# Vicky0522/TokensGen

Measured on AMD Instinct MI355X. Metric: DiT denoising steps/sec, CogVideoX-5B To2V 720x480 (CFG-batched 13-frame FIFO window: DiT fwd + CFG + 13 DPM updates), higher is better.
Workload: dtype bf16; 1 GPU; To2V FIFO window step, CogVideoX-5B 42 layers D=3072, 226 text + 17550 video + 480 vip tokens, CFG batch 2, DPM-solver++; layers=42, exchange=none

## Files before the change

include/tokensgen_hip.h:

```cpp
#ifndef TOKENSGEN_HIP_H
#define TOKENSGEN_HIP_H

#include <stdint.h>

#ifdef __cplusplus
extern "C" {
#endif
#if defined(__GNUC__)
#pragma GCC visibility push(default)
#endif

typedef struct ihipStream_t* hipStream_t;

#define TG_MAX_GROUPS 16

typedef struct tg_group_table {
    const void*    mod;
    long           mod_ld;
    long           mod_batch_stride;
    const uint8_t* tok_group;
    int32_t        row[TG_MAX_GROUPS];
    int32_t        shift_col[TG_MAX_GROUPS];
    int32_t        scale_col[TG_MAX_GROUPS];
    int32_t        gate_col[TG_MAX_GROUPS];
// ... 21 lines not shown

int tg_gemm_bf16_qkv(const void* A1, long strideA1, const void* W1, const void* bias1, void* C1, long strideC1, int M1, void* Vt1, long vt_ld1,
                     const void* A2, long strideA2, const void* W2, const void* bias2, void* C2, long strideC2, int M2, void* Vt2, long vt_ld2,
                     long lda, long ldw, long ldc, int N, int K, int batch, int v_col0, hipStream_t stream);

int tg_gemm_bf16_lora(const void* A, long lda, long strideA, const void* W, long ldw, const void* bias,
                      const void* T, long ldt, long strideT, const void* B, long ldb, float scale,
                      void* C, long ldc, long strideC, int M, int N, int K, int R, int batch, hipStream_t stream);

long tg_gemm_kernel(int M, int N, int K, long lda, long ldw);

int tg_adaln_modulate(const void* x, long ldx, long strideX, void* y, long ldy, long strideY,
                      const void* ln_weight, const void* ln_bias, float eps, int tokens, int dim, int batch,
                      int modulate, const tg_group_table* g, hipStream_t stream);

int tg_qk_layernorm_rope(void* x, long ld, long strideB, int tokens, int heads, int batch,
                         const void* ln_weight, const void* ln_bias, float eps,
                         int start0, int len0, const float* cos0, const float* sin0,
                         int start1, int len1, const float* cos1, const float* sin1, float out_scale, hipStream_t stream);

int tg_qk_layernorm_rope_pair(void* xq, void* xk, long ld, long strideB, int tokens, int heads, int batch,
                              const void* q_weight, const void* q_bias, const void* k_weight, const void* k_bias, float eps,
                              int start0, int len0, const float* cos0, const float* sin0,
                              int start1, int len1, const float* cos1, const float* sin1, float q_scale, float k_scale,
                              hipStream_t stream);

long tg_qk_kmax_ws_floats(int tokens, int heads, int batch);
int tg_qk_layernorm_rope_pair_kmax(void* xq, void* xk, long ld, long strideB, int tokens, int heads, int batch,
                                   const void* q_weight, const void* q_bias, const void* k_weight, const void* k_bias, float eps,
                                   int start0, int len0, const float* cos0, const float* sin0,
                                   int start1, int len1, const float* cos1, const float* sin1, float q_scale, float k_scale,
                                   float* k_norm2_max, float* ws, hipStream_t stream);

int tg_qk_layernorm_rope_pair_out(const void* xq, const void* xk, long ld, long strideB, void* yq, void* yk, long y_ld, long y_strideB, int tokens, int heads,
                                  int batch, const void* q_weight, const void* q_bias, const void* k_weight, const void* k_bias, float eps,
                                  int start0, int len0, const float* cos0, const float* sin0, int start1, int len1, const float* cos1, const float* sin1,
                                  float q_scale, float k_scale, float* k_norm2_max, float* ws, hipStream_t stream);

int tg_transpose_v(const void* v, long ld, long strideB, int key_start, int n_keys, int heads, int batch,
                   void* vt, long ldvt, hipStream_t stream);

int tg_attention_fwd(const void* q1, long q1_ld, long q1_strideB,
                     const void* k1, long k1_ld, long k1_strideB, const void* vt1, long vt1_ld, int nk1,
                     const void* q2, long q2_ld, long q2_strideB,
                     const void* k2, long k2_ld, long k2_strideB, const void* vt2, long vt2_ld, int nk2,
                     float seg2_scale, void* out, long out_ld, long out_strideB,
                     int nq, int heads, int batch, float scale, int k_prescaled, hipStream_t stream);

typedef struct tg_attn_segment {
    const void* q; long q_ld, q_strideB;
    const void* k; long k_ld, k_strideB;
    const void* vt; long vt_ld;
// ... 248 lines not shown
```

tokensgen_amd/csrc/norm.hip:

```cpp
#include "common.h"
#include "tokensgen_hip.h"

namespace {

template <int CHUNKS>
__global__ __launch_bounds__(256) void adaln_kernel(const bf16_t* __restrict__ x, long ldx, long sxb,
                                                    bf16_t* __restrict__ y, long ldy, long syb,
                                                    const bf16_t* __restrict__ w, const bf16_t* __restrict__ bvec,
                                                    float eps, int tokens, int dim, int batch, int modulate,
                                                    tg_group_table g) {
    const int lane = threadIdx.x & 63;
    const long row = (long)blockIdx.x * 4 + (threadIdx.x >> 6);
    if (row >= (long)tokens * batch) return;
    const int b = (int)(row / tokens), t = (int)(row % tokens);
    const bf16_t* xr = x + (long)b * sxb + (long)t * ldx;
    bf16_t* yr = y + (long)b * syb + (long)t * ldy;
    const int nvec = dim >> 3;

    uint4 raw[CHUNKS];
    float s = 0.f;
#pragma unroll
    for (int c = 0; c < CHUNKS; ++c) {
        const int v = c * 64 + lane;
        raw[c] = (v < nvec) ? *(const uint4*)(xr + v * 8) : uint4{0, 0, 0, 0};
// ... 39 lines not shown
            su[0] = sv.x; su[1] = sv.y; su[2] = sv.z; su[3] = sv.w;
            hu[0] = hv.x; hu[1] = hv.y; hu[2] = hv.z; hu[3] = hv.w;
        }
        uint32_t o[4];
#pragma unroll
        for (int i = 0; i < 4; ++i) {
            float lo = round_bf16((bf16lo_to_f32(u[i]) - mean) * rstd * bf16lo_to_f32(wu[i]) + bf16lo_to_f32(bu[i]));
            float hi = round_bf16((bf16hi_to_f32(u[i]) - mean) * rstd * bf16hi_to_f32(wu[i]) + bf16hi_to_f32(bu[i]));
            if (modulate) {
                lo = lo * (1.f + bf16lo_to_f32(su[i])) + bf16lo_to_f32(hu[i]);
                hi = hi * (1.f + bf16hi_to_f32(su[i])) + bf16hi_to_f32(hu[i]);
            }
            o[i] = pack_bf16x2(lo, hi);
        }
        *(uint4*)(yr + v * 8) = uint4{o[0], o[1], o[2], o[3]};
    }
}

__device__ __forceinline__ float qk_norm_rope_slice(const bf16_t* p, bf16_t* dstp, const bf16_t* __restrict__ w, const bf16_t* __restrict__ bvec, int part,
                                                    float eps, bool rope, const float (&c)[8], const float (&sv)[8], float out_scale, bool live) {
    const uint4 raw = *(const uint4*)p;
    const uint32_t u[4] = {raw.x, raw.y, raw.z, raw.w};
    float v[8];
    float s = 0.f;
#pragma unroll
    for (int i = 0; i < 4; ++i) {
        v[2 * i] = bf16lo_to_f32(u[i]);
        v[2 * i + 1] = bf16hi_to_f32(u[i]);
        s += v[2 * i] + v[2 * i + 1];
    }
// ... 95 lines not shown
            partial[((long)b * gridDim.x + blockIdx.x) * heads + threadIdx.x] = __uint_as_float(smax[threadIdx.x]);
    }
}

__global__ __launch_bounds__(256) void qk_kmax_finalize_kernel(const float* __restrict__ partial, int nblocks, int heads, float* __restrict__ kmax) {
    __shared__ float red[4];
    const int h = blockIdx.x, b = blockIdx.y;
    const float* src = partial + (long)b * nblocks * heads + h;
    float m = 0.f;
    for (int i = threadIdx.x; i < nblocks; i += 256) m = fmaxf(m, src[(long)i * heads]);
#pragma unroll
    for (int off = 32; off > 0; off >>= 1) m = fmaxf(m, __shfl_xor(m, off, 64));
    if ((threadIdx.x & 63) == 0) red[threadIdx.x >> 6] = m;
    __syncthreads();
    if (threadIdx.x == 0) kmax[b * heads + h] = fmaxf(fmaxf(red[0], red[1]), fmaxf(red[2], red[3]));
}

__global__ __launch_bounds__(256) void transpose_v_kernel(const bf16_t* __restrict__ v, long ld, long sb,
                                                          int key_start, int n_keys, int heads,
                                                          bf16_t* __restrict__ vt, long ldvt) {
    __shared__ bf16_t tile[64][64 + 8];
    const int kt = blockIdx.x, h = blockIdx.y, b = blockIdx.z;
    const int tid = threadIdx.x;
#pragma unroll
    for (int i = 0; i < 2; ++i) {
        const int idx = tid + i * 256;
        const int key = idx >> 3, ch = idx & 7;
        const int gk = kt * 64 + key;
        uint4 val{0, 0, 0, 0};
        if (gk < n_keys) val = *(const uint4*)(v + (long)b * sb + (long)(key_start + gk) * ld + h * 64 + ch * 8);
// ... 28 lines not shown
    if (g) gt = *g;
    const long rows = (long)tokens * batch;
    const dim3 grid((unsigned)((rows + 3) / 4)), block(256);
    const int chunks = (dim / 8 + 63) / 64;
#define TG_ADALN(C)                                                                                              \
    hipLaunchKernelGGL(adaln_kernel<C>, grid, block, 0, stream, (const bf16_t*)x, ldx, strideX, (bf16_t*)y, ldy,  \
                       strideY, (const bf16_t*)ln_weight, (const bf16_t*)ln_bias, eps, tokens, dim, batch, modulate, gt)
    if (chunks <= 1) TG_ADALN(1);
    else if (chunks <= 2) TG_ADALN(2);
    else if (chunks <= 4) TG_ADALN(4);
    else if (chunks <= 6) TG_ADALN(6);
    else if (chunks <= 8) TG_ADALN(8);
    else TG_ADALN(16);
#undef TG_ADALN
    TG_LAUNCH_CHECK("tg_adaln_modulate");
    return TG_OK;
}

static int qk_norm_rope_launch(void* xq, void* xk, long ld, long strideB, int tokens, int heads, int batch, const void* wq, const void* bq,
                               const void* wk, const void* bk, float eps, int start0, int len0, const float* cos0, const float* sin0,
                               int start1, int len1, const float* cos1, const float* sin1, float q_scale, float k_scale, hipStream_t stream,
                               float* k_norm2_max = nullptr, float* ws = nullptr, void* yq = nullptr, void* yk = nullptr, long yld = 0, long ysb = 0) {
    if (!yq) { yq = xq; yk = xk; yld = ld; ysb = strideB; }
    TG_REQUIRE(yld % 8 == 0 && ysb % 8 == 0 && tg_aligned16(yq) && (!xk || (yk && tg_aligned16(yk))), TG_ERR_ALIGN, "tg_qk_layernorm_rope: destination rows must be 16-byte aligned");
    TG_REQUIRE(xq && wq && bq && (!xk || (wk && bk)), TG_ERR_ARG, "tg_qk_layernorm_rope: null pointer");
    TG_REQUIRE(tokens > 0 && heads > 0 && batch > 0, TG_ERR_SHAPE, "tg_qk_layernorm_rope: bad shape");
    TG_REQUIRE(ld % 8 == 0 && strideB % 8 == 0 && tg_aligned16(xq) && (!xk || tg_aligned16(xk)), TG_ERR_ALIGN,
               "tg_qk_layernorm_rope: rows must be 16-byte aligned");
    TG_REQUIRE((len0 == 0 || (cos0 && sin0 && tg_aligned16(cos0) && tg_aligned16(sin0))) &&
               (len1 == 0 || (cos1 && sin1 && tg_aligned16(cos1) && tg_aligned16(sin1))), TG_ERR_ARG,
// ... 89 lines not shown
```

tokensgen_amd/kernels.py:

```python
import ctypes as C
import os

import torch

from . import lib as L

BF16 = torch.bfloat16


def _stream():
    return torch.cuda.current_stream().cuda_stream


def _chk(t, name, dtype=BF16):
    if not isinstance(t, torch.Tensor) or not t.is_cuda:
        raise RuntimeError(f"{name}: expected a GPU tensor (tokensgen_amd has no CPU fallback)")
    if t.dtype != dtype:
        raise TypeError(f"{name}: expected {dtype}, got {t.dtype}")
    if t.stride(-1) != 1:
        raise ValueError(f"{name}: innermost dimension must be contiguous")
    return t


def _p(t):
# ... 143 lines not shown
    name = f"gemm_qkv_M{M1}+{M2}_N{N}_K{Kd}" if two else f"gemm_qkv_M{M1}_N{N}_K{Kd}"
    L.check(_launch(name, L.load().tg_gemm_bf16_qkv, _p(a1), sa1, _p(w1), _p(bias1), _p(out1), sc1, M1, _p(vt1), ld1,
                    _p(a2) if two else None, sa2, _p(w2) if two else None, _p(bias2) if two else None, _p(out2) if two else None, sc2, M2,
                    _p(vt2) if two else None, ld2, lda, w1.stride(0), ldc, N, Kd, B, v_col0, _stream()), "tg_gemm_bf16_qkv")
    return out1, vt1


def adaln_modulate(x, out, ln_weight, ln_bias, eps, table=None):
    _chk(x, "x"); _chk(out, "out")
    B, T, D, ldx, sx = _bmk(x)
    _, _, _, ldy, sy = _bmk(out)
    L.check(_launch("adaln_modulate", L.load().tg_adaln_modulate, _p(x), ldx, sx, _p(out), ldy, sy, _p(ln_weight), _p(ln_bias), float(eps), T, D, B,
                                       1 if table is not None else 0, table.ref() if table is not None else None,
                                       _stream()), "tg_adaln_modulate")
    return out


def qk_layernorm_rope(x, heads, ln_weight, ln_bias, eps, seg0=None, seg1=None, out_scale=1.0):
    _chk(x, "x")
    B, T, HD, ld, sb = _bmk(x)
    assert HD == heads * 64

    def unpack(seg):
        if seg is None:
            return 0, 0, None, None
        start, (cos, sin) = seg
        _chk(cos, "cos", torch.float32); _chk(sin, "sin", torch.float32)
        assert cos.is_contiguous() and sin.is_contiguous() and cos.shape[-1] == 64
        return int(start), int(cos.shape[0]), cos, sin
    s0, l0, c0, n0 = unpack(seg0)
# ... 781 lines not shown
```

tokensgen_amd/lib.py:

```python
import ctypes as C
import os

_HERE = os.path.dirname(os.path.abspath(__file__))
LIB_PATH = os.environ.get("TG_LIB_PATH") or os.path.join(_HERE, "libtokensgen_hip.so")
TG_MAX_GROUPS = 16

EPI_BIAS, EPI_BIAS_GELU, EPI_BIAS_SILU, EPI_BIAS_GATE_RES = 0, 1, 2, 3
EPI_BIAS_KEEP_GELU, EPI_BIAS_MUL_GELU_GRAD = 4, 5


class GroupTable(C.Structure):
    _fields_ = [("mod", C.c_void_p), ("mod_ld", C.c_long), ("mod_batch_stride", C.c_long),
                ("tok_group", C.c_void_p), ("row", C.c_int32 * TG_MAX_GROUPS),
                ("shift_col", C.c_int32 * TG_MAX_GROUPS), ("scale_col", C.c_int32 * TG_MAX_GROUPS),
                ("gate_col", C.c_int32 * TG_MAX_GROUPS)]


_vp, _l, _i, _f, _d = C.c_void_p, C.c_long, C.c_int, C.c_float, C.c_double
PROTOTYPES = {
    "tg_gemm_bf16": [_vp, _l, _l, _vp, _l, _vp, _vp, _l, _l, _i, _i, _i, _i, _i, _vp, _l, _l, C.POINTER(GroupTable), _vp],
    "tg_gemm_bf16_pair": [_vp, _l, _vp, _vp, _vp, _l, _i, _vp, _l, _vp, _vp, _vp, _l, _i, _l, _l, _l, _i, _i, _i, _i, _vp],
    "tg_gemm_bf16_qkv": [_vp, _l, _vp, _vp, _vp, _l, _i, _vp, _l, _vp, _l, _vp, _vp, _vp, _l, _i, _vp, _l, _l, _l, _l, _i, _i, _i, _i, _vp],
    "tg_gemm_bf16_lora": [_vp, _l, _l, _vp, _l, _vp, _vp, _l, _l, _vp, _l, _f, _vp, _l, _l, _i, _i, _i, _i, _i, _vp],
    "tg_adaln_modulate": [_vp, _l, _l, _vp, _l, _l, _vp, _vp, _f, _i, _i, _i, _i, C.POINTER(GroupTable), _vp],
    "tg_qk_layernorm_rope": [_vp, _l, _l, _i, _i, _i, _vp, _vp, _f, _i, _i, _vp, _vp, _i, _i, _vp, _vp, _f, _vp],
    "tg_qk_layernorm_rope_pair": [_vp, _vp, _l, _l, _i, _i, _i, _vp, _vp, _vp, _vp, _f, _i, _i, _vp, _vp, _i, _i, _vp, _vp, _f, _f, _vp],
    "tg_qk_layernorm_rope_pair_kmax": [_vp, _vp, _l, _l, _i, _i, _i, _vp, _vp, _vp, _vp, _f, _i, _i, _vp, _vp, _i, _i, _vp, _vp, _f, _f, _vp, _vp, _vp],
    "tg_qk_layernorm_rope_pair_out": [_vp, _vp, _l, _l, _vp, _vp, _l, _l, _i, _i, _i, _vp, _vp, _vp, _vp, _f, _i, _i, _vp, _vp, _i, _i, _vp, _vp, _f, _f, _vp, _vp, _vp],
    "tg_transpose_v": [_vp, _l, _l, _i, _i, _i, _i, _vp, _l, _vp],
    "tg_attention_fwd": [_vp, _l, _l, _vp, _l, _l, _vp, _l, _i, _vp, _l, _l, _vp, _l, _l, _vp, _l, _i, _f, _vp, _l, _l,
                         _i, _i, _i, _f, _i, _vp],
    "tg_attention_fwd_multi": [_vp, _i, _i, _i, _f, _i, _vp, _vp],
    "tg_attention_bwd": [_vp, _l, _l, _vp, _l, _l, _vp, _l, _l, _vp, _l, _l, _vp, _l, _l, _vp, _l, _l, _vp, _l, _l, _vp, _l, _l,
                         _i, _i, _i, _i, _f, _i, _vp, _vp, _vp],
    "tg_attention_bwd_ex": [_vp, _l, _l, _vp, _l, _l, _vp, _l, _l, _vp, _l, _l, _vp, _l, _l, _vp, _l, _l, _vp, _l, _l, _vp, _l, _l,
                            _i, _i, _i, _i, _f, _i, _vp, _vp, _i, _vp, _vp],
    "tg_attention_bwd_multi": [_vp, _i, _i, _i, _i, _vp, _vp],
    "tg_attention_bwd_probe": [_vp, _l, _vp],
    "tg_attention_bwd_probe_verdict": [_vp, _l],
# ... 153 lines not shown
class ColsumItem(C.Structure):
    _fields_ = [("src", C.c_void_p), ("ld", C.c_long), ("rows", C.c_int), ("cols", C.c_int), ("src_is_f32", C.c_int)]


TG_ACCUM_MAX, TG_COLSUM_MAX = 48, 16


class Adamw8bitRow(C.Structure):
    _fields_ = [("offset", C.c_long), ("numel", C.c_long), ("state", C.c_long), ("first_block", C.c_long), ("kind", C.c_int), ("clipped", C.c_int)]


ADAMW8BIT_FP32, ADAMW8BIT_BLOCKWISE = 0, 1
PRODIGY_STATE_DOUBLES = 8


class AttnSegment(C.Structure):
    _fields_ = [("q", C.c_void_p), ("q_ld", C.c_long), ("q_strideB", C.c_long),
                ("k", C.c_void_p), ("k_ld", C.c_long), ("k_strideB", C.c_long),
                ("vt", C.c_void_p), ("vt_ld", C.c_long), ("nk", C.c_int), ("k_norm2_max", C.c_void_p)]


class AttnProblem(C.Structure):
    _fields_ = [("seg", AttnSegment * 2), ("nseg", C.c_int), ("seg2_scale", C.c_float),
                ("out", C.c_void_p), ("out_ld", C.c_long), ("out_strideB", C.c_long), ("nq", C.c_int),
                ("seg2_scale_batch", C.POINTER(C.c_float))]


class AttnWorkspace(C.Structure):
    _fields_ = [("retry", C.c_void_p), ("retry_ints", C.c_long), ("split", C.c_void_p), ("split_floats", C.c_long)]
```

tokensgen_amd/transformer.py:

```python
import json
import math
import os
from types import SimpleNamespace

import torch
from torch import nn

from . import kernels as K
from . import lib as L

BF16 = torch.bfloat16


class Transformer2DModelOutput:
    def __init__(self, sample):
        self.sample = sample


class VideoIPAdapterCogVideoXAttnProcessor2_0(nn.Module):

    def __init__(self, scale=1.0, num_tokens=None):
        super().__init__()
        self.scale = scale
        self.num_tokens = num_tokens
# ... 377 lines not shown

    def _workspace(self, B, Nt, Nv, Np, Fm):
        key = (B, Nt, Nv, Np, Fm)
        ws = self._ws.get(key)
        if ws is not None:
            return ws
        D, H = self.inner_dim, self.config.num_attention_heads
        N1, N = Nt + Nv, Nt + Nv + Np
        dev = self._device
        e = lambda *s: torch.empty(*s, dtype=BF16, device=dev)
        ws = SimpleNamespace()
        ws.X, ws.Xn, ws.AO = e(B, N, D), e(B, N, D), e(B, N, D)
        ws.QKV = e(B, N1, 3 * D)
        ws.FF = e(B, N, 4 * D)
        ws.Vt1 = e(B, H, 64, _pad_to(N1, 64))
        ws.kmax1 = torch.zeros(B, H, dtype=torch.float32, device=dev)
        ws.kmax2 = torch.zeros(B, H, dtype=torch.float32, device=dev)
        ws.kmax_ws = K.kmax_workspace(N, H, B, dev)
        ws.retry = K.AttnRetry(N1, Np, H, B, dev)
        if Np:
            ws.QKVv = e(B, N, 3 * D)
            ws.Vt2 = e(B, H, 64, _pad_to(Np, 64))
            ws.Vt3 = e(B, H, 64, _pad_to(N, 64))
        per, out_base, total = self._mod_cols()
        ws.mod = e(B, Fm, _pad_to(total, 128))
        ws.sin = e(B * Fm, D)
        ws.t1 = e(B * Fm, self.config.time_embed_dim)
        ws.semb = e(B * Fm, self.config.time_embed_dim)
        ws.patches = torch.zeros(B, Nv, self._fused["patch.w"].shape[1], dtype=BF16, device=dev)
        ws.po = e(B, Nv, self._fused["proj_out.w"].shape[0])
        hw = Nv // Fm if Fm > 1 else Nv
        tg = torch.empty(N, dtype=torch.uint8)
        tg[:Nt] = Fm
# ... 18 lines not shown
        sc = [main + D] * Fm + [main + 4 * D, vip + D]
        ga = [main + 2 * D] * Fm + [main + 5 * D, vip + 2 * D]
        return K.GroupTable(ws.mod, ws.tok_group, rows, sh, sc, ga)

    def _run_block(self, i, ws, B, Nt, Nv, Np, Fm, rope, vrope, crope):
        c, D, H = self.config, self.inner_dim, self.config.num_attention_heads
        F = self._fused
        X = ws.X
        N1, N = Nt + Nv, Nt + Nv + Np
        use_vip = Np > 0
        sm_scale = 1.0 / math.sqrt(64)
        blk = self.transformer_blocks[i]
        p = f"l{i}."
        ln = F[p + "ln"]
        t1 = self._tables(ws, i, Fm, 1)
        K.adaln_modulate(X[:, :N1], ws.Xn[:, :N1], ln[0], ln[1], c.norm_eps, t1)
        if use_vip:
            vln = F[p + "vln"]
            K.adaln_modulate(X[:, N1:], ws.Xn[:, N1:], vln[0], vln[1], c.norm_eps, t1.offset(N1))
        self._attn_core(i, ws, B, Nt, Nv, Np, rope, vrope, crope)
        K.gemm(ws.AO, F[p + "out.w"], F[p + "out.b"], X, L.EPI_BIAS_GATE_RES, residual=X, gate=t1)
        t2 = self._tables(ws, i, Fm, 2)
        K.adaln_modulate(X[:, :N1], ws.Xn[:, :N1], ln[2], ln[3], c.norm_eps, t2)
        if use_vip:
            K.adaln_modulate(X[:, N1:], ws.Xn[:, N1:], vln[2], vln[3], c.norm_eps, t2.offset(N1))
        K.gemm(ws.Xn, F[p + "ff1.w"], F[p + "ff1.b"], ws.FF, L.EPI_BIAS_GELU)
        K.gemm(ws.FF, F[p + "ff2.w"], F[p + "ff2.b"], X, L.EPI_BIAS_GATE_RES, residual=X, gate=t2)


    def _attn_core(self, i, ws, B, Nt, Nv, Np, rope, vrope, crope):
        D, H = self.inner_dim, self.config.num_attention_heads
        F = self._fused
        N1, N = Nt + Nv, Nt + Nv + Np
        use_vip = Np > 0
        sm_scale = 1.0 / math.sqrt(64)
        blk = self.transformer_blocks[i]
        p = f"l{i}."
        paired = use_vip and K.gemm_pair_supported(N1, N, 3 * D, D)
        pad64 = lambda n: (n + 63) // 64 * 64
        vt2_view_ok = N1 % 8 == 0 and N1 + pad64(Np) <= pad64(N)
        fused_vt = K.gemm_qkv_supported(N1, 3 * D, D, 2 * D) and (not use_vip or vt2_view_ok)
        qn = F[p + "qknorm"]
        kscale = sm_scale * 1.4426950408889634
        if fused_vt and use_vip:
            K.gemm_qkv(ws.Xn[:, :N1], F[p + "qkv.w"], F[p + "qkv.b"], ws.QKV, ws.Vt1, ws.Xn, F[p + "vqkv.w"], F[p + "vqkv.b"], ws.QKVv, ws.Vt3)
        elif fused_vt:
            K.gemm_qkv(ws.Xn[:, :N1], F[p + "qkv.w"], F[p + "qkv.b"], ws.QKV, ws.Vt1)
        elif paired:
            K.gemm_pair(ws.Xn[:, :N1], F[p + "qkv.w"], F[p + "qkv.b"], ws.QKV, ws.Xn, F[p + "vqkv.w"], F[p + "vqkv.b"], ws.QKVv, L.EPI_BIAS)
        else:
            K.gemm(ws.Xn[:, :N1], F[p + "qkv.w"], F[p + "qkv.b"], ws.QKV, L.EPI_BIAS)
        fast = self._attn_fast(ws) if getattr(ws, "retry", None) is not None else False
        K.qk_layernorm_rope_pair(ws.QKV[:, :, :D], ws.QKV[:, :, D:2 * D], H, qn[0], qn[1], qn[2], qn[3], 1e-6, (Nt, rope), k_scale=kscale,
                                 kmax=ws.kmax1 if fast else None, kmax_ws=ws.kmax_ws if fast else None)
        if not fused_vt:
            K.transpose_v(ws.QKV[:, :, 2 * D:], H, 0, N1, ws.Vt1)
        if use_vip:
            if not paired and not fused_vt:
                K.gemm(ws.Xn, F[p + "vqkv.w"], F[p + "vqkv.b"], ws.QKVv, L.EPI_BIAS)
            vqn = F[p + "vqknorm"]
            K.qk_layernorm_rope_pair(ws.QKVv[:, :, :D], ws.QKVv[:, :, D:2 * D], H, vqn[0], vqn[1], vqn[2], vqn[3], 1e-6, (Nt, vrope),
                                     (N1, crope), k_scale=kscale, kmax=ws.kmax2 if fast else None, kmax_ws=ws.kmax_ws if fast else None)
            if not fused_vt:
                K.transpose_v(ws.QKVv[:, :, 2 * D:], H, 0, N, ws.Vt3)
            if vt2_view_ok and N1 + pad64(Np) <= ws.Vt3.shape[3]:
                vt2 = ws.Vt3[:, :, :, N1:]
            else:
                vt2 = K.transpose_v(ws.QKVv[:, :, 2 * D:], H, N1, Np, ws.Vt2)
            s = blk.attn1.processor.scale
            sl = [float(v) for v in s] if isinstance(s, (list, tuple)) else [float(s)]
            sl = [float(torch.tensor(v, dtype=torch.float32).to(BF16)) for v in sl]
            s_batch = sl if (len(sl) == B and len(set(sl)) > 1) else None
            s = sl[0]
            km1, km2 = (ws.kmax1, ws.kmax2) if fast else (None, None)
            K.attention_multi(dict(q1=ws.QKV[:, :, :D], k1=ws.QKV[:, :, D:2 * D], vt1=ws.Vt1, nk1=N1, out=ws.AO[:, :N1],
                                   q2=ws.QKVv[:, :N1, :D], k2=ws.QKVv[:, N1:, D:2 * D], vt2=vt2, nk2=Np, seg2_scale=s, kmax1=km1, kmax2=km2, seg2_scale_batch=s_batch),
                              dict(q1=ws.QKVv[:, N1:, :D], k1=ws.QKVv[:, :, D:2 * D], vt1=ws.Vt3, nk1=N, out=ws.AO[:, N1:], kmax1=km2),
                              H, sm_scale, k_prescaled=True, retry=ws.retry if fast else None, split=getattr(ws.retry, "split", None))
        elif fast:
            K.attention_multi(dict(q1=ws.QKV[:, :, :D], k1=ws.QKV[:, :, D:2 * D], vt1=ws.Vt1, nk1=N1, out=ws.AO[:, :N1], kmax1=ws.kmax1), None,
                              H, sm_scale, k_prescaled=True, retry=ws.retry)
        else:
            K.attention(ws.QKV[:, :, :D], ws.QKV[:, :, D:2 * D], ws.Vt1, N1, ws.AO[:, :N1], H, sm_scale, k_prescaled=True)

    @torch.no_grad()
    def attention_op(self, i, hidden_states, encoder_hidden_states, image_rotary_emb=None, vip_image_rotary_emb=None,
                     vip_condition_rotary_emb=None):
        dev = self._device
        B, Nv, D = hidden_states.shape
        Np = self.vip_length if self.transformer_blocks[i].use_vip else 0
        Nt = encoder_hidden_states.shape[1] - Np
        N1, N = Nt + Nv, Nt + Nv + Np
        H = self.config.num_attention_heads
        if image_rotary_emb is None or (Np and (vip_image_rotary_emb is None or vip_condition_rotary_emb is None)):
            raise ValueError("rotary tables are required (CogVideoX-5B attention)")
        e = lambda *sh: torch.empty(*sh, dtype=BF16, device=dev)
        ws = SimpleNamespace(Xn=e(B, N, D), QKV=e(B, N1, 3 * D), Vt1=e(B, H, 64, _pad_to(N1, 64)), AO=e(B, N, D))
        ws.kmax1 = torch.zeros(B, H, dtype=torch.float32, device=dev)
        ws.kmax2 = torch.zeros(B, H, dtype=torch.float32, device=dev)
        ws.kmax_ws, ws.retry = K.kmax_workspace(N, H, B, dev), K.AttnRetry(N1, Np, H, B, dev)
        ws.Xn[:, :Nt] = encoder_hidden_states[:, :Nt].to(dev, BF16)
        ws.Xn[:, Nt:N1] = hidden_states.to(dev, BF16)
        f32 = lambda t: tuple(x.to(dev, torch.float32).contiguous() for x in t)
        vr = cr = None
        if Np:
            ws.Xn[:, N1:] = encoder_hidden_states[:, Nt:].to(dev, BF16)
            ws.QKVv, ws.Vt2, ws.Vt3 = e(B, N, 3 * D), e(B, H, 64, _pad_to(Np, 64)), e(B, H, 64, _pad_to(N, 64))
            vr, cr = f32(vip_image_rotary_emb), f32(vip_condition_rotary_emb)
        self._attn_core(i, ws, B, Nt, Nv, Np, f32(image_rotary_emb), vr, cr)
        out = e(B, N, D)
        F = self._fused
        K.gemm(ws.AO, F[f"l{i}.out.w"], F[f"l{i}.out.b"], out, L.EPI_BIAS)
        return out[:, Nt:N1], torch.cat([out[:, :Nt], out[:, N1:]], dim=1)

    @torch.no_grad()
# ... 79 lines not shown
```

Measured before the change: 1.626 steps/s.

## Merge split AdaLN launches and batch both QK-norm/RoPE problems into one kernel

Result: no change. 1.625 steps/s (median of 2 runs) (-0.0%).

```diff
diff --git a/include/tokensgen_hip.h b/include/tokensgen_hip.h
--- a/include/tokensgen_hip.h
+++ b/include/tokensgen_hip.h
@@ -59,6 +59,10 @@
                       const void* ln_weight, const void* ln_bias, float eps, int tokens, int dim, int batch,
                       int modulate, const tg_group_table* g, hipStream_t stream);
 
+int tg_adaln_modulate_rows2(const void* x, long ldx, long strideX, void* y, long ldy, long strideY, const void* w0, const void* b0,
+                            const void* w1, const void* b1, float eps, int tokens, int split, int dim, int batch,
+                            const tg_group_table* g, hipStream_t stream);
+
 int tg_qk_layernorm_rope(void* x, long ld, long strideB, int tokens, int heads, int batch,
                          const void* ln_weight, const void* ln_bias, float eps,
                          int start0, int len0, const float* cos0, const float* sin0,
@@ -81,6 +85,27 @@
                                   int batch, const void* q_weight, const void* q_bias, const void* k_weight, const void* k_bias, float eps,
                                   int start0, int len0, const float* cos0, const float* sin0, int start1, int len1, const float* cos1, const float* sin1,
                                   float q_scale, float k_scale, float* k_norm2_max, float* ws, hipStream_t stream);
+
+typedef struct tg_qk_problem {
+    void*        q;
+    void*        k;
+    long         ld, strideB;
+    int          tokens;
+    const void*  q_weight;
+    const void*  q_bias;
+    const void*  k_weight;
+    const void*  k_bias;
+    int          start0, len0;
+    const float* cos0;
+    const float* sin0;
+    int          start1, len1;
+    const float* cos1;
+    const float* sin1;
+    float        q_scale, k_scale;
+    float*       k_norm2_max;
+    float*       k_norm2_max_clear;
+} tg_qk_problem;
+int tg_qk_layernorm_rope_multi(const tg_qk_problem* problems, int nproblems, int heads, int batch, float eps, hipStream_t stream);
 
 int tg_transpose_v(const void* v, long ld, long strideB, int key_start, int n_keys, int heads, int batch,
                    void* vt, long ldvt, hipStream_t stream);
diff --git a/tokensgen_amd/csrc/norm.hip b/tokensgen_amd/csrc/norm.hip
--- a/tokensgen_amd/csrc/norm.hip
+++ b/tokensgen_amd/csrc/norm.hip
@@ -1,3 +1,5 @@
+#include <algorithm>
+
 #include "common.h"
 #include "tokensgen_hip.h"
 
@@ -77,6 +79,95 @@
             o[i] = pack_bf16x2(lo, hi);
         }
         *(uint4*)(yr + v * 8) = uint4{o[0], o[1], o[2], o[3]};
+    }
+}
+
+template <int CHUNKS>
+__device__ __forceinline__ void adaln_row(const bf16_t* xr, bf16_t* yr, const bf16_t* w, const bf16_t* bvec, const bf16_t* scale, const bf16_t* shift,
+                                          float eps, int dim, int lane) {
+    const int nvec = dim >> 3;
+    uint4 raw[CHUNKS];
+    float s = 0.f;
+#pragma unroll
+    for (int c = 0; c < CHUNKS; ++c) {
+        const int v = c * 64 + lane;
+        raw[c] = (v < nvec) ? *(const uint4*)(xr + v * 8) : uint4{0, 0, 0, 0};
+        const uint32_t u[4] = {raw[c].x, raw[c].y, raw[c].z, raw[c].w};
+#pragma unroll
+        for (int i = 0; i < 4; ++i) s += bf16lo_to_f32(u[i]) + bf16hi_to_f32(u[i]);
+    }
+    const float mean = wave_sum(s) / dim;
+    float q = 0.f;
+#pragma unroll
+    for (int c = 0; c < CHUNKS; ++c) {
+        const int v = c * 64 + lane;
+        if (v < nvec) {
+            const uint32_t u[4] = {raw[c].x, raw[c].y, raw[c].z, raw[c].w};
+#pragma unroll
+            for (int i = 0; i < 4; ++i) {
+                const float a = bf16lo_to_f32(u[i]) - mean, c2 = bf16hi_to_f32(u[i]) - mean;
+                q += a * a + c2 * c2;
+            }
+        }
+    }
+    const float rstd = rsqrtf(wave_sum(q) / dim + eps);
+#pragma unroll
+    for (int c = 0; c < CHUNKS; ++c) {
+        const int v = c * 64 + lane;
+        if (v >= nvec) continue;
+        const uint32_t u[4] = {raw[c].x, raw[c].y, raw[c].z, raw[c].w};
+        const uint4 wv = *(const uint4*)(w + v * 8), bv = *(const uint4*)(bvec + v * 8);
+        const uint4 sv = *(const uint4*)(scale + v * 8), hv = *(const uint4*)(shift + v * 8);
+        const uint32_t wu[4] = {wv.x, wv.y, wv.z, wv.w}, bu[4] = {bv.x, bv.y, bv.z, bv.w};
+        const uint32_t su[4] = {sv.x, sv.y, sv.z, sv.w}, hu[4] = {hv.x, hv.y, hv.z, hv.w};
+        uint32_t o[4];
+#pragma unroll
+        for (int i = 0; i < 4; ++i) {
+            float lo = round_bf16((bf16lo_to_f32(u[i]) - mean) * rstd * bf16lo_to_f32(wu[i]) + bf16lo_to_f32(bu[i]));
+            float hi = round_bf16((bf16hi_to_f32(u[i]) - mean) * rstd * bf16hi_to_f32(wu[i]) + bf16hi_to_f32(bu[i]));
+            lo = lo * (1.f + bf16lo_to_f32(su[i])) + bf16lo_to_f32(hu[i]);
+            hi = hi * (1.f + bf16hi_to_f32(su[i])) + bf16hi_to_f32(hu[i]);
+            o[i] = pack_bf16x2(lo, hi);
+        }
+        *(uint4*)(yr + v * 8) = uint4{o[0], o[1], o[2], o[3]};
+    }
+}
+
+template <int CHUNKS, int ROWS>
+__global__ __launch_bounds__(256) void adaln_rows_kernel(const bf16_t* __restrict__ x, long ldx, long sxb, bf16_t* __restrict__ y, long ldy, long syb,
+                                                         const bf16_t* __restrict__ w0, const bf16_t* __restrict__ b0, const bf16_t* __restrict__ w1,
+                                                         const bf16_t* __restrict__ b1, float eps, int tokens, int split, int dim, int batch,
+                                                         tg_group_table g) {
+    __shared__ uint4 staged[4][CHUNKS * 64];
+    const int lane = threadIdx.x & 63, wave = threadIdx.x >> 6;
+    const int per_batch = (tokens + 4 * ROWS - 1) / (4 * ROWS);
+    const int b = (int)blockIdx.x / per_batch, t0 = ((int)blockIdx.x % per_batch) * (4 * ROWS);
+    const int t1 = min(t0 + 4 * ROWS, tokens);
+    const bf16_t* modb = (const bf16_t*)g.mod + (long)b * g.mod_batch_stride;
+    const int nvec = dim >> 3;
+    const int key0 = g.tok_group[t0] * 2 + (t0 >= split);
+    {
+        const int gi = key0 >> 1;
+        const bf16_t* base = modb + (long)g.row[gi] * g.mod_ld;
+        const bf16_t* src = wave == 0 ? ((key0 & 1) ? w1 : w0) : wave == 1 ? ((key0 & 1) ? b1 : b0) : wave == 2 ? base + g.scale_col[gi] : base + g.shift_col[gi];
+#pragma unroll
+        for (int c = 0; c < CHUNKS; ++c) {
+            const int v = c * 64 + lane;
+            if (v < nvec) staged[wave][v] = *(const uint4*)(src + v * 8);
+        }
+    }
+    __syncthreads();
+#pragma unroll 1
+    for (int t = t0 + wave; t < t1; t += 4) {
+        const bf16_t* xr = x + (long)b * sxb + (long)t * ldx;
+        bf16_t* yr = y + (long)b * syb + (long)t * ldy;
+        const int gi = g.tok_group[t], half = t >= split;
+        if (gi * 2 + half == key0) {
+            adaln_row<CHUNKS>(xr, yr, (const bf16_t*)staged[0], (const bf16_t*)staged[1], (const bf16_t*)staged[2], (const bf16_t*)staged[3], eps, dim, lane);
+        } else {
+            const bf16_t* base = modb + (long)g.row[gi] * g.mod_ld;
+            adaln_row<CHUNKS>(xr, yr, half ? w1 : w0, half ? b1 : b0, base + g.scale_col[gi], base + g.shift_col[gi], eps, dim, lane);
+        }
     }
 }
 
@@ -202,6 +293,83 @@
     if ((threadIdx.x & 63) == 0) red[threadIdx.x >> 6] = m;
     __syncthreads();
     if (threadIdx.x == 0) kmax[b * heads + h] = fmaxf(fmaxf(red[0], red[1]), fmaxf(red[2], red[3]));
+}
+
+constexpr int QK_MULTI_THREADS = 256;
+constexpr int QK_MULTI_ROUNDS = 2;
+struct QkMultiParams {
+    tg_qk_problem p[2];
+    int wgs[2];
+    int heads;
+    float eps;
+};
+
+template <int HPG, bool STATS>
+__global__ __launch_bounds__(QK_MULTI_THREADS) void qk_norm_rope_multi_kernel(QkMultiParams P) {
+    __shared__ unsigned smax[STATS ? 128 : 1];
+    const int tid = threadIdx.x;
+    const int pi = (int)blockIdx.x >= P.wgs[0] ? 1 : 0;
+    const tg_qk_problem& pr = P.p[pi];
+    const int j = (int)blockIdx.x - (pi ? P.wgs[0] : 0), nw = P.wgs[pi];
+    const int b = blockIdx.y, heads = P.heads, tokens = pr.tokens;
+    const int hgroups = heads / HPG;
+    const long rows = (long)tokens * hgroups;
+    const int part = tid & 7;
+    if (STATS) {
+        if (tid < 128) smax[tid] = 0u;
+        if (j == 0 && pr.k_norm2_max_clear && tid < heads) pr.k_norm2_max_clear[(long)b * heads + tid] = 0.f;
+        __syncthreads();
+    }
+    bf16_t* xq = (bf16_t*)pr.q + (long)b * pr.strideB;
+    bf16_t* xk = (bf16_t*)pr.k + (long)b * pr.strideB;
+    const bf16_t* wq = (const bf16_t*)pr.q_weight;
+    const bf16_t* bq = (const bf16_t*)pr.q_bias;
+    const bf16_t* wk = (const bf16_t*)pr.k_weight;
+    const bf16_t* bk = (const bf16_t*)pr.k_bias;
+    const long ld = pr.ld;
+    const int start0 = pr.start0, len0 = pr.len0, start1 = pr.start1, len1 = pr.len1;
+    const float q_scale = pr.q_scale, k_scale = pr.k_scale, eps = P.eps;
+    for (long base = (long)j * (QK_MULTI_THREADS / 8) + (tid >> 6) * 8; base < rows; base += (long)nw * (QK_MULTI_THREADS / 8)) {
+        const long rowid = base + ((tid & 63) >> 3);
+        const bool live = rowid < rows;
+        const long rid = live ? rowid : rows - 1;
+        const int h0 = (int)(rid % hgroups) * HPG;
+        const int t = (int)(rid / hgroups);
+        const float* cs = nullptr;
+        const float* sn = nullptr;
+        if (t >= start0 && t < start0 + len0) {
+            cs = pr.cos0 + (long)(t - start0) * 64 + part * 8;
+            sn = pr.sin0 + (long)(t - start0) * 64 + part * 8;
+        } else if (t >= start1 && t < start1 + len1) {
+            cs = pr.cos1 + (long)(t - start1) * 64 + part * 8;
+            sn = pr.sin1 + (long)(t - start1) * 64 + part * 8;
+        }
+        float c[8] = {0.f, 0.f, 0.f, 0.f, 0.f, 0.f, 0.f, 0.f}, sv[8] = {0.f, 0.f, 0.f, 0.f, 0.f, 0.f, 0.f, 0.f};
+        if (cs) {
+            const float4 c0 = *(const float4*)cs, c1 = *(const float4*)(cs + 4);
+            const float4 s0 = *(const float4*)sn, s1 = *(const float4*)(sn + 4);
+            c[0] = c0.x; c[1] = c0.y; c[2] = c0.z; c[3] = c0.w; c[4] = c1.x; c[5] = c1.y; c[6] = c1.z; c[7] = c1.w;
+            sv[0] = s0.x; sv[1] = s0.y; sv[2] = s0.z; sv[3] = s0.w; sv[4] = s1.x; sv[5] = s1.y; sv[6] = s1.z; sv[7] = s1.w;
+        }
+#pragma unroll
+        for (int hh = 0; hh < HPG; ++hh) {
+            const long off = (long)t * ld + (h0 + hh) * 64 + part * 8;
+            qk_norm_rope_slice(xq + off, xq + off, wq, bq, part, eps, cs != nullptr, c, sv, q_scale, live);
+            float ss = qk_norm_rope_slice(xk + off, xk + off, wk, bk, part, eps, cs != nullptr, c, sv, k_scale, live);
+            if (STATS) {
+                ss += __shfl_xor(ss, 1, 64); ss += __shfl_xor(ss, 2, 64); ss += __shfl_xor(ss, 4, 64);
+                if (part == 0 && live) atomicMax(&smax[h0 + hh], __float_as_uint(ss));
+            }
+        }
+    }
+    if (STATS) {
+        __syncthreads();
+        if (tid < heads) {
+            unsigned* dst = (unsigned*)pr.k_norm2_max + (long)b * heads + tid;
+            const unsigned v = smax[tid];
+            if (v > __hip_atomic_load(dst, __ATOMIC_RELAXED, __HIP_MEMORY_SCOPE_AGENT)) atomicMax(dst, v);
+        }
+    }
 }
 
 __global__ __launch_bounds__(256) void transpose_v_kernel(const bf16_t* __restrict__ v, long ld, long sb,
@@ -260,6 +428,85 @@
     else TG_ADALN(16);
 #undef TG_ADALN
     TG_LAUNCH_CHECK("tg_adaln_modulate");
+    return TG_OK;
+}
+
+constexpr int ADALN_ROWS = 2;
+
+extern "C" int tg_adaln_modulate_rows2(const void* x, long ldx, long strideX, void* y, long ldy, long strideY, const void* w0, const void* b0,
+                                       const void* w1, const void* b1, float eps, int tokens, int split, int dim, int batch,
+                                       const tg_group_table* g, hipStream_t stream) {
+    TG_REQUIRE(x && y && w0 && b0 && g && g->mod && g->tok_group, TG_ERR_ARG, "tg_adaln_modulate_rows2: null pointer");
+    TG_REQUIRE(tokens > 0 && batch > 0 && dim > 0 && dim % 8 == 0 && dim <= 4096 && split >= 0 && split <= tokens, TG_ERR_SHAPE,
+               "tg_adaln_modulate_rows2: bad shape tokens=%d split=%d dim=%d batch=%d (dim <= 4096)", tokens, split, dim, batch);
+    TG_REQUIRE(split == tokens || (w1 && b1), TG_ERR_ARG, "tg_adaln_modulate_rows2: rows past split need their own affine");
+    TG_REQUIRE(ldx % 8 == 0 && ldy % 8 == 0 && strideX % 8 == 0 && strideY % 8 == 0 && g->mod_ld % 8 == 0 && g->mod_batch_stride % 8 == 0 &&
+               tg_aligned16(x) && tg_aligned16(y) && tg_aligned16(w0) && tg_aligned16(b0) && tg_aligned16(w1) && tg_aligned16(b1) && tg_aligned16(g->mod),
+               TG_ERR_ALIGN, "tg_adaln_modulate_rows2: rows and vectors must be 16-byte aligned");
+    const long wgs = (long)((tokens + 4 * ADALN_ROWS - 1) / (4 * ADALN_ROWS)) * batch;
+    TG_REQUIRE(wgs < (1L << 31), TG_ERR_SHAPE, "tg_adaln_modulate_rows2: too many rows");
+    const dim3 grid((unsigned)wgs), block(256);
+    const int chunks = (dim / 8 + 63) / 64;
+#define TG_ADALN_ROWS(C)                                                                                                                   \
+    hipLaunchKernelGGL((adaln_rows_kernel<C, ADALN_ROWS>), grid, block, 0, stream, (const bf16_t*)x, ldx, strideX, (bf16_t*)y, ldy, strideY, \
+                       (const bf16_t*)w0, (const bf16_t*)b0, (const bf16_t*)w1, (const bf16_t*)b1, eps, tokens, split, dim, batch, *g)
+    if (chunks <= 1) TG_ADALN_ROWS(1);
+    else if (chunks <= 2) TG_ADALN_ROWS(2);
+    else if (chunks <= 4) TG_ADALN_ROWS(4);
+    else if (chunks <= 6) TG_ADALN_ROWS(6);
+    else TG_ADALN_ROWS(8);
+#undef TG_ADALN_ROWS
+    TG_LAUNCH_CHECK("tg_adaln_modulate_rows2");
+    return TG_OK;
+}
+
+extern "C" int tg_qk_layernorm_rope_multi(const tg_qk_problem* problems, int nproblems, int heads, int batch, float eps, hipStream_t stream) {
+    TG_REQUIRE(problems, TG_ERR_ARG, "tg_qk_layernorm_rope_multi: null pointer");
+    TG_REQUIRE((nproblems == 1 || nproblems == 2) && heads > 0 && batch > 0 && batch <= 65535, TG_ERR_SHAPE,
+               "tg_qk_layernorm_rope_multi: bad shape nproblems=%d heads=%d batch=%d", nproblems, heads, batch);
+    const bool stats = problems[0].k_norm2_max != nullptr;
+    TG_REQUIRE(!stats || heads <= 128, TG_ERR_SHAPE, "tg_qk_layernorm_rope_multi: heads=%d > 128", heads);
+    const int hpg = heads % 4 == 0 ? 4 : heads % 2 == 0 ? 2 : 1;
+    QkMultiParams P{};
+    P.heads = heads;
+    P.eps = eps;
+    long rows[2] = {0, 0};
+    for (int i = 0; i < nproblems; ++i) {
+        const tg_qk_problem& p = problems[i];
+        TG_REQUIRE(p.q && p.k && p.q_weight && p.q_bias && p.k_weight && p.k_bias, TG_ERR_ARG, "tg_qk_layernorm_rope_multi: null pointer (problem %d)", i);
+        TG_REQUIRE(p.tokens > 0, TG_ERR_SHAPE, "tg_qk_layernorm_rope_multi: bad shape (problem %d)", i);
+        TG_REQUIRE(p.ld % 8 == 0 && p.strideB % 8 == 0 && tg_aligned16(p.q) && tg_aligned16(p.k) && tg_aligned16(p.q_weight) && tg_aligned16(p.q_bias) &&
+                   tg_aligned16(p.k_weight) && tg_aligned16(p.k_bias), TG_ERR_ALIGN, "tg_qk_layernorm_rope_multi: rows must be 16-byte aligned (problem %d)", i);
+        TG_REQUIRE((p.len0 == 0 || (p.cos0 && p.sin0 && tg_aligned16(p.cos0) && tg_aligned16(p.sin0))) &&
+                   (p.len1 == 0 || (p.cos1 && p.sin1 && tg_aligned16(p.cos1) && tg_aligned16(p.sin1))), TG_ERR_ARG,
+                   "tg_qk_layernorm_rope_multi: rope tables missing or unaligned (problem %d)", i);
+        TG_REQUIRE(p.len0 >= 0 && p.len1 >= 0 && p.start0 >= 0 && p.start1 >= 0 && p.start0 + p.len0 <= p.tokens && p.start1 + p.len1 <= p.tokens,
+                   TG_ERR_SHAPE, "tg_qk_layernorm_rope_multi: rope segment outside the token range (problem %d)", i);
+        TG_REQUIRE(!p.k_norm2_max == !stats, TG_ERR_ARG, "tg_qk_layernorm_rope_multi: k_norm2_max on every problem or on none");
+        TG_REQUIRE(!p.k_norm2_max_clear || (stats && p.k_norm2_max_clear != p.k_norm2_max), TG_ERR_ARG,
+                   "tg_qk_layernorm_rope_multi: k_norm2_max_clear needs k_norm2_max and must be another buffer");
+        P.p[i] = p;
+        rows[i] = (long)p.tokens * (heads / hpg);
+    }
+    using Kernel = void (*)(QkMultiParams);
+    static const Kernel kernels[2][3] = {{qk_norm_rope_multi_kernel<4, false>, qk_norm_rope_multi_kernel<2, false>, qk_norm_rope_multi_kernel<1, false>},
+                                         {qk_norm_rope_multi_kernel<4, true>, qk_norm_rope_multi_kernel<2, true>, qk_norm_rope_multi_kernel<1, true>}};
+    static int resident[2][3];
+    const int ki = hpg == 4 ? 0 : hpg == 2 ? 1 : 2;
+    const Kernel kernel = kernels[stats][ki];
+    if (resident[stats][ki] <= 0) {
+        int n = 0;
+        (void)hipOccupancyMaxActiveBlocksPerMultiprocessor(&n, kernel, QK_MULTI_THREADS, 0);
+        resident[stats][ki] = std::max(n, 1);
+    }
+    const long budget = std::max(1L, (long)QK_MULTI_ROUNDS * resident[stats][ki] * tg_device_cus() / batch);
+    const long rows_step = QK_MULTI_THREADS / 8;
+    for (int i = 0; i < nproblems; ++i) {
+        const long share = std::max(1L, (budget * rows[i] + (rows[0] + rows[1]) / 2) / (rows[0] + rows[1]));
+        P.wgs[i] = (int)std::min(share, (rows[i] + rows_step - 1) / rows_step);
+    }
+    hipLaunchKernelGGL(kernel, dim3((unsigned)(P.wgs[0] + P.wgs[1]), (unsigned)batch), dim3(QK_MULTI_THREADS), 0, stream, P);
+    TG_LAUNCH_CHECK("tg_qk_layernorm_rope_multi");
     return TG_OK;
 }
 
diff --git a/tokensgen_amd/kernels.py b/tokensgen_amd/kernels.py
--- a/tokensgen_amd/kernels.py
+++ b/tokensgen_amd/kernels.py
@@ -181,6 +181,60 @@
                                        1 if table is not None else 0, table.ref() if table is not None else None,
                                        _stream()), "tg_adaln_modulate")
     return out
+
+
+def adaln_modulate_rows2(x, out, w0, b0, w1, b1, eps, split, table):
+    _chk(x, "x"); _chk(out, "out")
+    B, T, D, ldx, sx = _bmk(x)
+    _, _, _, ldy, sy = _bmk(out)
+    L.check(_launch("adaln_modulate_rows2", L.load().tg_adaln_modulate_rows2, _p(x), ldx, sx, _p(out), ldy, sy, _p(w0), _p(b0), _p(w1), _p(b1), float(eps),
+                    T, int(split), D, B, table.ref(), _stream()), "tg_adaln_modulate_rows2")
+    return out
+
+
+class KmaxBuffers:
+
+    def __init__(self, problems, batch, heads, device):
+        self.buf = torch.zeros(2, problems, batch, heads, dtype=torch.float32, device=device)
+        self.i = 0
+
+    @property
+    def cur(self):
+        return self.buf[self.i]
+
+    def flip(self):
+        self.i ^= 1
+        return self.buf[self.i], self.buf[self.i ^ 1]
+
+
+def qk_layernorm_rope_multi(problems, heads, eps, kmax=None):
+    assert 1 <= len(problems) <= 2
+    arr = (L.QkProblem * len(problems))()
+    cur, clear = kmax.flip() if kmax is not None else (None, None)
+    B = None
+    for i, pr in enumerate(problems):
+        xq, xk = pr["xq"], pr["xk"]
+        _chk(xq, "xq"); _chk(xk, "xk")
+        Bi, T, HD, ld, sb = _bmk(xq)
+        assert HD == heads * 64 and _bmk(xk) == (Bi, T, HD, ld, sb) and B in (None, Bi)
+        B = Bi
+        c = arr[i]
+        c.q, c.k, c.ld, c.strideB, c.tokens = _p(xq), _p(xk), ld, sb, T
+        c.q_weight, c.q_bias, c.k_weight, c.k_bias = _p(pr["q_weight"]), _p(pr["q_bias"]), _p(pr["k_weight"]), _p(pr["k_bias"])
+        for j, seg in enumerate((pr.get("seg0"), pr.get("seg1"))):
+            if seg is None:
+                continue
+            start, (cos, sin) = seg
+            _chk(cos, "cos", torch.float32); _chk(sin, "sin", torch.float32)
+            assert cos.is_contiguous() and sin.is_contiguous() and cos.shape[-1] == 64
+            setattr(c, f"start{j}", int(start)); setattr(c, f"len{j}", int(cos.shape[0]))
+            setattr(c, f"cos{j}", _p(cos)); setattr(c, f"sin{j}", _p(sin))
+        c.q_scale, c.k_scale = float(pr.get("q_scale", 1.0)), float(pr.get("k_scale", 1.0))
+        if kmax is not None:
+            assert cur.shape[0] > i and cur.shape[1:] == (B, heads)
+            c.k_norm2_max, c.k_norm2_max_clear = _p(cur[i]), _p(clear[i])
+    L.check(_launch("qk_layernorm_rope_multi", L.load().tg_qk_layernorm_rope_multi, C.cast(arr, C.c_void_p), len(problems), heads, B, float(eps), _stream()),
+            "tg_qk_layernorm_rope_multi")
 
 
 def qk_layernorm_rope(x, heads, ln_weight, ln_bias, eps, seg0=None, seg1=None, out_scale=1.0):
diff --git a/tokensgen_amd/lib.py b/tokensgen_amd/lib.py
--- a/tokensgen_amd/lib.py
+++ b/tokensgen_amd/lib.py
@@ -23,6 +23,8 @@
     "tg_gemm_bf16_qkv": [_vp, _l, _vp, _vp, _vp, _l, _i, _vp, _l, _vp, _l, _vp, _vp, _vp, _l, _i, _vp, _l, _l, _l, _l, _i, _i, _i, _i, _vp],
     "tg_gemm_bf16_lora": [_vp, _l, _l, _vp, _l, _vp, _vp, _l, _l, _vp, _l, _f, _vp, _l, _l, _i, _i, _i, _i, _i, _vp],
     "tg_adaln_modulate": [_vp, _l, _l, _vp, _l, _l, _vp, _vp, _f, _i, _i, _i, _i, C.POINTER(GroupTable), _vp],
+    "tg_adaln_modulate_rows2": [_vp, _l, _l, _vp, _l, _l, _vp, _vp, _vp, _vp, _f, _i, _i, _i, _i, C.POINTER(GroupTable), _vp],
+    "tg_qk_layernorm_rope_multi": [_vp, _i, _i, _i, _f, _vp],
     "tg_qk_layernorm_rope": [_vp, _l, _l, _i, _i, _i, _vp, _vp, _f, _i, _i, _vp, _vp, _i, _i, _vp, _vp, _f, _vp],
     "tg_qk_layernorm_rope_pair": [_vp, _vp, _l, _l, _i, _i, _i, _vp, _vp, _vp, _vp, _f, _i, _i, _vp, _vp, _i, _i, _vp, _vp, _f, _f, _vp],
     "tg_qk_layernorm_rope_pair_kmax": [_vp, _vp, _l, _l, _i, _i, _i, _vp, _vp, _vp, _vp, _f, _i, _i, _vp, _vp, _i, _i, _vp, _vp, _f, _f, _vp, _vp, _vp],
@@ -206,6 +208,14 @@
 PRODIGY_STATE_DOUBLES = 8
 
 
+class QkProblem(C.Structure):
+    _fields_ = [("q", C.c_void_p), ("k", C.c_void_p), ("ld", C.c_long), ("strideB", C.c_long), ("tokens", C.c_int),
+                ("q_weight", C.c_void_p), ("q_bias", C.c_void_p), ("k_weight", C.c_void_p), ("k_bias", C.c_void_p),
+                ("start0", C.c_int), ("len0", C.c_int), ("cos0", C.c_void_p), ("sin0", C.c_void_p),
+                ("start1", C.c_int), ("len1", C.c_int), ("cos1", C.c_void_p), ("sin1", C.c_void_p),
+                ("q_scale", C.c_float), ("k_scale", C.c_float), ("k_norm2_max", C.c_void_p), ("k_norm2_max_clear", C.c_void_p)]
+
+
 class AttnSegment(C.Structure):
     _fields_ = [("q", C.c_void_p), ("q_ld", C.c_long), ("q_strideB", C.c_long),
                 ("k", C.c_void_p), ("k_ld", C.c_long), ("k_strideB", C.c_long),
diff --git a/tokensgen_amd/transformer.py b/tokensgen_amd/transformer.py
--- a/tokensgen_amd/transformer.py
+++ b/tokensgen_amd/transformer.py
@@ -415,9 +415,7 @@
         ws.QKV = e(B, N1, 3 * D)
         ws.FF = e(B, N, 4 * D)
         ws.Vt1 = e(B, H, 64, _pad_to(N1, 64))
-        ws.kmax1 = torch.zeros(B, H, dtype=torch.float32, device=dev)
-        ws.kmax2 = torch.zeros(B, H, dtype=torch.float32, device=dev)
-        ws.kmax_ws = K.kmax_workspace(N, H, B, dev)
+        ws.kmax = K.KmaxBuffers(2, B, H, dev)
         ws.retry = K.AttnRetry(N1, Np, H, B, dev)
         if Np:
             ws.QKVv = e(B, N, 3 * D)
@@ -466,16 +464,12 @@
         p = f"l{i}."
         ln = F[p + "ln"]
         t1 = self._tables(ws, i, Fm, 1)
-        K.adaln_modulate(X[:, :N1], ws.Xn[:, :N1], ln[0], ln[1], c.norm_eps, t1)
-        if use_vip:
-            vln = F[p + "vln"]
-            K.adaln_modulate(X[:, N1:], ws.Xn[:, N1:], vln[0], vln[1], c.norm_eps, t1.offset(N1))
+        vln = F[p + "vln"] if use_vip else (None,) * 4
+        K.adaln_modulate_rows2(X, ws.Xn, ln[0], ln[1], vln[0], vln[1], c.norm_eps, N1, t1)
         self._attn_core(i, ws, B, Nt, Nv, Np, rope, vrope, crope)
         K.gemm(ws.AO, F[p + "out.w"], F[p + "out.b"], X, L.EPI_BIAS_GATE_RES, residual=X, gate=t1)
         t2 = self._tables(ws, i, Fm, 2)
-        K.adaln_modulate(X[:, :N1], ws.Xn[:, :N1], ln[2], ln[3], c.norm_eps, t2)
-        if use_vip:
-            K.adaln_modulate(X[:, N1:], ws.Xn[:, N1:], vln[2], vln[3], c.norm_eps, t2.offset(N1))
+        K.adaln_modulate_rows2(X, ws.Xn, ln[2], ln[3], vln[2], vln[3], c.norm_eps, N1, t2)
         K.gemm(ws.Xn, F[p + "ff1.w"], F[p + "ff1.b"], ws.FF, L.EPI_BIAS_GELU)
         K.gemm(ws.FF, F[p + "ff2.w"], F[p + "ff2.b"], X, L.EPI_BIAS_GATE_RES, residual=X, gate=t2)
 
@@ -503,16 +497,18 @@
         else:
             K.gemm(ws.Xn[:, :N1], F[p + "qkv.w"], F[p + "qkv.b"], ws.QKV, L.EPI_BIAS)
         fast = self._attn_fast(ws) if getattr(ws, "retry", None) is not None else False
-        K.qk_layernorm_rope_pair(ws.QKV[:, :, :D], ws.QKV[:, :, D:2 * D], H, qn[0], qn[1], qn[2], qn[3], 1e-6, (Nt, rope), k_scale=kscale,
-                                 kmax=ws.kmax1 if fast else None, kmax_ws=ws.kmax_ws if fast else None)
+        if use_vip and not paired and not fused_vt:
+            K.gemm(ws.Xn, F[p + "vqkv.w"], F[p + "vqkv.b"], ws.QKVv, L.EPI_BIAS)
+        qk = [dict(xq=ws.QKV[:, :, :D], xk=ws.QKV[:, :, D:2 * D], q_weight=qn[0], q_bias=qn[1], k_weight=qn[2], k_bias=qn[3], seg0=(Nt, rope), k_scale=kscale)]
+        if use_vip:
+            vqn = F[p + "vqknorm"]
+            qk.append(dict(xq=ws.QKVv[:, :, :D], xk=ws.QKVv[:, :, D:2 * D], q_weight=vqn[0], q_bias=vqn[1], k_weight=vqn[2], k_bias=vqn[3], seg0=(Nt, vrope),
+                           seg1=(N1, crope), k_scale=kscale))
+        K.qk_layernorm_rope_multi(qk, H, 1e-6, kmax=ws.kmax if fast else None)
+        kmax1, kmax2 = (ws.kmax.cur[0], ws.kmax.cur[1]) if fast else (None, None)
         if not fused_vt:
             K.transpose_v(ws.QKV[:, :, 2 * D:], H, 0, N1, ws.Vt1)
         if use_vip:
-            if not paired and not fused_vt:
-                K.gemm(ws.Xn, F[p + "vqkv.w"], F[p + "vqkv.b"], ws.QKVv, L.EPI_BIAS)
-            vqn = F[p + "vqknorm"]
-            K.qk_layernorm_rope_pair(ws.QKVv[:, :, :D], ws.QKVv[:, :, D:2 * D], H, vqn[0], vqn[1], vqn[2], vqn[3], 1e-6, (Nt, vrope),
-                                     (N1, crope), k_scale=kscale, kmax=ws.kmax2 if fast else None, kmax_ws=ws.kmax_ws if fast else None)
             if not fused_vt:
                 K.transpose_v(ws.QKVv[:, :, 2 * D:], H, 0, N, ws.Vt3)
             if vt2_view_ok and N1 + pad64(Np) <= ws.Vt3.shape[3]:
@@ -524,13 +520,13 @@
             sl = [float(torch.tensor(v, dtype=torch.float32).to(BF16)) for v in sl]
             s_batch = sl if (len(sl) == B and len(set(sl)) > 1) else None
             s = sl[0]
-            km1, km2 = (ws.kmax1, ws.kmax2) if fast else (None, None)
+            km1, km2 = kmax1, kmax2
             K.attention_multi(dict(q1=ws.QKV[:, :, :D], k1=ws.QKV[:, :, D:2 * D], vt1=ws.Vt1, nk1=N1, out=ws.AO[:, :N1],
                                    q2=ws.QKVv[:, :N1, :D], k2=ws.QKVv[:, N1:, D:2 * D], vt2=vt2, nk2=Np, seg2_scale=s, kmax1=km1, kmax2=km2, seg2_scale_batch=s_batch),
                               dict(q1=ws.QKVv[:, N1:, :D], k1=ws.QKVv[:, :, D:2 * D], vt1=ws.Vt3, nk1=N, out=ws.AO[:, N1:], kmax1=km2),
                               H, sm_scale, k_prescaled=True, retry=ws.retry if fast else None, split=getattr(ws.retry, "split", None))
         elif fast:
-            K.attention_multi(dict(q1=ws.QKV[:, :, :D], k1=ws.QKV[:, :, D:2 * D], vt1=ws.Vt1, nk1=N1, out=ws.AO[:, :N1], kmax1=ws.kmax1), None,
+            K.attention_multi(dict(q1=ws.QKV[:, :, :D], k1=ws.QKV[:, :, D:2 * D], vt1=ws.Vt1, nk1=N1, out=ws.AO[:, :N1], kmax1=kmax1), None,
                               H, sm_scale, k_prescaled=True, retry=ws.retry)
         else:
             K.attention(ws.QKV[:, :, :D], ws.QKV[:, :, D:2 * D], ws.Vt1, N1, ws.AO[:, :N1], H, sm_scale, k_prescaled=True)
@@ -548,9 +544,7 @@
             raise ValueError("rotary tables are required (CogVideoX-5B attention)")
         e = lambda *sh: torch.empty(*sh, dtype=BF16, device=dev)
         ws = SimpleNamespace(Xn=e(B, N, D), QKV=e(B, N1, 3 * D), Vt1=e(B, H, 64, _pad_to(N1, 64)), AO=e(B, N, D))
-        ws.kmax1 = torch.zeros(B, H, dtype=torch.float32, device=dev)
-        ws.kmax2 = torch.zeros(B, H, dtype=torch.float32, device=dev)
-        ws.kmax_ws, ws.retry = K.kmax_workspace(N, H, B, dev), K.AttnRetry(N1, Np, H, B, dev)
+        ws.kmax, ws.retry = K.KmaxBuffers(2, B, H, dev), K.AttnRetry(N1, Np, H, B, dev)
         ws.Xn[:, :Nt] = encoder_hidden_states[:, :Nt].to(dev, BF16)
         ws.Xn[:, Nt:N1] = hidden_states.to(dev, BF16)
         f32 = lambda t: tuple(x.to(dev, torch.float32).contiguous() for x in t)
```
